# valette/FROG

Measured on AMD Instinct MI355X. Metric: registration iterations/sec (linear+deformable), higher is better.
Workload: dtype f32

## Files before the change

frog_amd/csrc/device/ctx.h:

```cpp
#pragma once

#include <hip/hip_runtime.h>

#include <cstdint>
#include <cstdio>
#include <cstring>
#include <string>
#include <memory>
#include <vector>

#include "../../../include/frog_hip.h"
#include "dev_buf.h"
#include "switches.h"

namespace frog {

extern thread_local std::string g_last_error;

inline int fail(int code, const std::string &msg)
{
    g_last_error = msg;
    return code;
}

#define FROG_HIP_CHECK(expr)                                                            \
    do {                                                                                \
        hipError_t e_ = (expr);                                                         \
        if (e_ != hipSuccess)                                                           \
            return ::frog::fail(FROG_E_HIP, std::string(#expr) + ": " + hipGetErrorString(e_)); \
    } while (0)

constexpr int SC_ENERGY = 0, SC_COUNT = 1;
constexpr int SC_OVERSIZE = 2;
constexpr int SC_LIST_STALE = 3;
constexpr int N_SCALARS = 4;
constexpr int HS_BBOX = 4, HS_SEQ = 7, HS_DOUBLES = 8;
struct ScalarHandoff {
    enum How { NONE, BY_KERNEL, BY_COPY, BY_COPY_SYNC } how = NONE;
    double seq = 0.0;
};
struct StepScalars {
    double E, n_oversize;
};


constexpr int TILE_POINTS = 256;
constexpr int N_XCD = 8;
constexpr int MAX_SUBPASS = 8;
constexpr int MAX_GROUPS = N_XCD * MAX_SUBPASS;
constexpr int REC_CHUNK = 128;
__host__ __device__ inline size_t group_sum_index(uint32_t group, uint32_t point, uint32_t own_points)
// ... 137 lines not shown
    frog::DevBuf<double> img_energy;
    frog::DevBuf<unsigned int> energy_ticket;
    double *h_energy = nullptr;
    double *h_energy_dev = nullptr;
    uint64_t scalar_seq = 0;

    bool deformable = false;
    frog::GridGeom geom{};
    frog::DevBuf<float4> coeff;
    frog::DevBuf<float4> grad;
    frog::DevBuf<float4> gradf;
    frog::DevBuf<float4> grad_spare;
    frog::DevBuf<uint32_t> lat_mask;
    frog::DevBuf<uint32_t> lat_inactive;
    frog::DevBuf<float4> ucoeff, ugrad, ugrad_spare;
    void commit_proposal() { coeff.swap(grad); ucoeff.swap(ugrad); coeff_zero = false; }
    void speculate_commit()
    {
        spec_coeff_zero = coeff_zero;
        coeff.swap(grad); grad.swap(grad_spare);
        ucoeff.swap(ugrad); ugrad.swap(ugrad_spare);
        coeff_zero = false;
    }
    void rollback_speculation()
    {
        grad.swap(grad_spare); coeff.swap(grad);
        ugrad.swap(ugrad_spare); ucoeff.swap(ugrad);
        coeff_zero = spec_coeff_zero;
    }
    frog::DevBuf<double> gridsum;
    frog::DevBuf<uint32_t> perm;
    frog::DevBuf<uint32_t> key_ptr;
    frog::DevBuf<uint32_t> key_cursor;
    frog::DevBuf<uint32_t> key_counts, brick_ptr_scratch, scan_sums;
    frog::DevBuf<unsigned char> scatter_blocks;
    frog::DevBuf<unsigned char> scatter_blocks_tmp;
    frog::DevBuf<uint32_t> len_hist;
    uint32_t n_scatter_blocks = 0;
    frog::DevBuf<float> bounds_scratch;
    frog::DevBuf<unsigned int> stray;
    uint32_t stray_parity = 0;
    bool centered_in_a = false;
    frog::DevBuf<long long> img_counts;
// ... 1 lines not shown
    std::vector<frog::GridRecord> grids;
    uint32_t n_hard = 0;
    float hard_weight2 = 0;
    frog::DevBuf<uint32_t> hl_point, hl_ptr, hl_partner;
    frog::DevBuf<double> hl_partial;
    frog::DevBuf<uint32_t> perm_tmp;
    frog::DevBuf<uint32_t> perm_key;
    frog::DevBuf<float4> scatter_stage;
    frog::DevBuf<uint32_t> brick_slot_ptr;
    frog::DevBuf<float4> extract_tmp;
    frog::DevBuf<uint32_t> subset_idx;
    frog::DevBuf<float> subset_out;
    std::vector<float4> h_res_sums, h_res_pos;
    bool res_valid = false;
    bool xyz2_fresh = false;
    float pending_alpha = 0;
    int phase = 0;

    bool ref_order = false;
    double create_s[3] = { 0, 0, 0 };
    int create_selections = 0;
    bool created = false;
    int lattice_reallocs = 0;
    bool two_collectives = false;
    bool finish_deformable = false;
    bool speculated = false;
    bool spec_coeff_zero = false;
    frog::ScalarHandoff pending;
    frog::DevBuf<uint32_t> ref_own;
    frog::DevBuf<float> ref_w, ref_d;
// ... 72 lines not shown
```

frog_amd/csrc/device/frog_hip.hip:

```cpp

#include "ctx.h"
#include <hip/hip_ext.h>
#include "prep.h"
#include "k_links.hip.h"
#include "k_stats.hip.h"
#include "k_grid.hip.h"
#include "k_comm.hip.h"
#include "k_cull.hip.h"
#include "k_ransac.hip.h"
#include "k_reforder.hip.h"
#include "k_refchain.hip.h"
#include "similarity.h"

#include <atomic>
#include <chrono>
#include <cmath>
#include <cstdlib>
#include <random>
#include <limits>
#include <new>

namespace frog {
thread_local std::string g_last_error;
constexpr int BOUNDS_BLOCKS = 256;
// ... 308 lines not shown
        ctx->pos_b_stale = false;
    }
    return FROG_OK;
}

static int post_step_scalars(frog_ctx *ctx, ScalarHandoff::How how, ScalarHandoff &h)
{
    h.how = how == ScalarHandoff::BY_KERNEL && !ctx->h_energy_dev ? ScalarHandoff::BY_COPY : how;
    h.seq = h.how == ScalarHandoff::BY_KERNEL ? (double)(++ctx->scalar_seq) : 0.0;
    if (h.how == ScalarHandoff::BY_KERNEL) return FROG_OK;
    FROG_HIP_CHECK(hipMemcpyAsync(ctx->h_energy, ctx->energy.p, N_SCALARS * sizeof(double), hipMemcpyDeviceToHost, ctx->stream));
    if (h.how == ScalarHandoff::BY_COPY) FROG_HIP_CHECK(hipEventRecord(ctx->energy_copied, ctx->stream));
    return FROG_OK;
}

static int await_step_scalars(frog_ctx *ctx, ScalarHandoff &h, StepScalars &out)
{
    const ScalarHandoff posted = h;
    h = ScalarHandoff{};
    volatile double *hs = ctx->h_energy;
    if (posted.how == ScalarHandoff::BY_KERNEL) {
        const auto t0 = std::chrono::steady_clock::now();
        unsigned spins = 0;
        while (hs[HS_SEQ] != posted.seq) {
            __builtin_ia32_pause();
            if ((++spins & 0xFFFFu) == 0u && std::chrono::steady_clock::now() - t0 > std::chrono::seconds(20)) {
                FROG_HIP_CHECK(hipStreamSynchronize(ctx->stream));
                if (hs[HS_SEQ] != posted.seq) return fail(FROG_E_HIP, "the step's scalars never arrived");
            }
        }
        std::atomic_thread_fence(std::memory_order_acquire);
    } else if (posted.how == ScalarHandoff::BY_COPY) FROG_HIP_CHECK(hipEventSynchronize(ctx->energy_copied));
    else FROG_HIP_CHECK(hipStreamSynchronize(ctx->stream));
    if (ctx->h_energy[SC_LIST_STALE] > 0) ctx->cull_need_build = true;
    out.E = std::sqrt(ctx->h_energy[SC_ENERGY] / ctx->h_energy[SC_COUNT]);
    out.n_oversize = ctx->h_energy[SC_OVERSIZE];
    return FROG_OK;
}

static bool step_rejected(const frog_ctx *ctx, double n_oversize) { return ctx->opt.guarantee_diffeomorphism && n_oversize > 0; }

static void record_displacement(frog_ctx *ctx, const P3 *out, bool measured, uint32_t n_blocks)
{
    if (measured) ctx->disp_n = ctx->disp_own_n = n_blocks;
    ctx->disp_others = false;
    ctx->disp_current = measured && out == ctx->pos2.p;
// ... 574 lines not shown
        for (uint32_t i = 0; i < c->n_owned(); i++) std::memcpy(&st[(size_t)i * MT_WORDS], x, sizeof x);
        CREATE_CHECK(c->mt_state.upload(st, s));
    }
    return FROG_OK;
}

static int create_solver_buffers(frog_ctx *c, const CreateClock &clock)
{
    hipStream_t s = c->stream;
    std::vector<double> hm((size_t)c->nI * 16, 0.0);
    for (uint32_t i = 0; i < c->nI; i++) for (int k = 0; k < 4; k++) hm[(size_t)i * 16 + 5 * k] = 1.0;
    CREATE_CHECK(c->mat.upload(hm, s));
    CREATE_CHECK(c->energy.alloc(4));
    CREATE_CHECK(c->energy_blocks.alloc(2 * ENERGY_BLOCKS));
    CREATE_CHECK(c->img_energy.alloc(2 * (size_t)std::max(1u, c->n_owned())));
    CREATE_CHECK(c->energy_ticket.alloc(2));
    CREATE_CHECK(hipMemsetAsync(c->energy_ticket.p, 0, 2 * sizeof(unsigned int), s));
    CREATE_CHECK(hipMemsetAsync(c->energy.p, 0, c->energy.bytes(), s));
    CREATE_CHECK(c->stray.alloc(3));
    CREATE_CHECK(hipMemsetAsync(c->stray.p, 0, 3 * sizeof(unsigned int), s));
    CREATE_CHECK(c->bounds_scratch.alloc((size_t)BOUNDS_BLOCKS * 6 + 6));
    em_derive_kernel<<<div_up(c->nI, 256), 256, 0, s>>>(c->em.p, c->emd.p, c->emf.p, c->nI, c->fast_theta());
    CREATE_CHECK(hipGetLastError());
    resolve_modes(c);
    CREATE_CHECK(c->cut_now.alloc(c->nI));
    CREATE_CHECK(c->lin_listed.alloc(1));
    CREATE_CHECK(hipMemsetAsync(c->lin_listed.p, 0, sizeof(unsigned long long), s));
    if (c->cull_enabled && (c->opt.inlier_threshold >= 1e-3f || c->cull_linear) && c->n_tiles > 0) {
        if (int rc_ = cull_allocate(c)) return rc_;
    }
    stats_publish_kernel<<<dim3(div_up(c->nI, 64), 2), 64, 0, s>>>(c->em.p, c->emd.p, c->emf.p, c->nI, c->opt.inlier_threshold, c->fast_theta(), c->cut_now.p, 1);
    CREATE_CHECK(hipGetLastError());
// ... 69 lines not shown
            (void)hipGetLastError();
        }
        if (c->retired_arena.alloc(arena) != hipSuccess) (void)hipGetLastError();
        c->retired_used = 0;
    }
    clock.lap("+ lattices allocated");
}

static void resolve_kernels(frog_ctx *c, const CreateClock &clock)
{
    const void *kernels[] = {
        (const void *)sweep_kernel<SWEEP_DEFORMABLE, true, false, false, false>, (const void *)sweep_kernel<SWEEP_DEFORMABLE, true, false, true, false>,
        (const void *)sweep_kernel<SWEEP_DEFORMABLE, true, false, false, true>, (const void *)sweep_kernel<SWEEP_COUNT, true, false, false, false>,
        (const void *)scatter_kernel, (const void *)lattice_step_kernel<true>, (const void *)lattice_step_kernel<false>,
        (const void *)transform_bspline_tile_kernel<float>, (const void *)transform_bspline_kernel<float>, (const void *)transform_bspline_kernel<float, 2>, (const void *)transform_zero_lattice_kernel,
        (const void *)cp_center_kernel, (const void *)bounds_kernel, (const void *)bounds_final_kernel, (const void *)zero_buffers_kernel,
        (const void *)brick_count_kernel, (const void *)brick_place_kernel, (const void *)cell_order_kernel, (const void *)brick_chunks_kernel,
        (const void *)scan_block_sums_kernel, (const void *)scan_of_sums_kernel, (const void *)scan_apply_kernel,
        (const void *)block_fill_kernel, (const void *)block_len_base_kernel, (const void *)block_sort_kernel,
        (const void *)cull_list_cutoff_kernel, (const void *)cull_allow_kernel, (const void *)cull_validate_kernel, (const void *)cull_disp_kernel,
        (const void *)count_reduce_kernel, (const void *)combine_groups_kernel, (const void *)energy_reduce_kernel,
        (const void *)lattice_step_kernel<true, LS_CPB_SMALL>, (const void *)lattice_step_kernel<false, LS_CPB_SMALL>,
        (const void *)stats_publish_kernel, (const void *)cull_allow_validate_kernel, (const void *)cull_count_kernel,
        (const void *)sweep_kernel<SWEEP_LINEAR, true, false, true, false>, (const void *)sweep_kernel<SWEEP_LINEAR, true, false, false, false>,
    };
    for (const void *k : kernels) { hipFuncAttributes fa; (void)hipFuncGetAttributes(&fa, k); }
    (void)hipGetLastError();
    scratch_warm_kernel<<<1, 64, 0, c->stream>>>(c->stray.p, 0);
    (void)hipGetLastError();
    (void)hipStreamSynchronize(c->stream);
    clock.lap("+ kernels resolved, stream idle");
// ... 153 lines not shown
            const float a = (float)((double)(1 - cpos) * lo + (double)cpos * hi);
            anchors[3 * (size_t)i + j] = a;
            if (i < nI - ctx->nf) average[j] += a / (float)(nI - ctx->nf);
        }
    std::vector<double> hm((size_t)nI * 16, 0.0);
    for (uint32_t i = 0; i < nI; i++) {
        for (int k = 0; k < 4; k++) hm[(size_t)i * 16 + 5 * k] = 1.0;
        for (int j = 0; j < 3; j++) hm[(size_t)i * 16 + 4 * j + 3] = (double)(average[j] - anchors[3 * (size_t)i + j]);
    }
    FROG_HIP_CHECK(hipMemcpyAsync(ctx->mat.p, hm.data(), hm.size() * sizeof(double), hipMemcpyHostToDevice, ctx->stream));
    FROG_HIP_CHECK(hipStreamSynchronize(ctx->stream));
    { const int rc = join_setup(ctx); if (rc) return rc; }
    ctx->deformable = false;
    ctx->phase = 0;
    ctx->xyz2_fresh = false; ctx->res_valid = false;
    ctx->disp_current = false; ctx->disp_spec = false; ctx->disp_others = false;
    ctx->cull_need_build = true; ctx->cull_check_due = true;
    stats_publish_kernel<<<dim3(div_up(ctx->nI, 64), 2), 64, 0, ctx->stream>>>(ctx->em.p, ctx->emd.p, ctx->emf.p, ctx->nI, ctx->opt.inlier_threshold, ctx->fast_theta(), ctx->cut_now.p, 1);
    FROG_HIP_CHECK(hipGetLastError());
    return FROG_OK;
}

static int launch_transform(frog_ctx *ctx, P3 *out, int apply, bool after_step = false, double scalar_seq = 0.0, double *trailer = nullptr)
{
    double *host_scalars = scalar_seq != 0.0 ? ctx->h_energy_dev : nullptr;
    const uint32_t n = ctx->own_pt_end - ctx->own_pt_begin;
    if (!n) return FROG_OK;
    Span span(ctx, FROG_K_TRANSFORM);
    if (!ctx->deformable) {
        const bool with_disp = cull_active_linear(ctx) && ctx->cull_lin_builds > 0 && !ctx->cull_need_build && ctx->pos2_snap.p;
        transform_linear_kernel<<<div_up(n, 256), 256, 0, ctx->stream>>>(ctx->pos.p, out, ctx->mat.p,
                                                                        ctx->own_pt_begin, ctx->own_pt_end, apply,
                                                                        with_disp ? ctx->pos2_snap.p : nullptr, ctx->disp_part.p,
                                                                        ctx->disp_allow.p, ctx->cull_state.p, ctx->energy.p,
                                                                        host_scalars, scalar_seq, trailer);
        trailer = nullptr;
        record_displacement(ctx, out, with_disp, div_up(n, 256));
    } else if (ctx->coeff_zero && !after_step) {
        record_displacement(ctx, out, false, 0);
        transform_zero_lattice_kernel<<<div_up(n, 256), 256, 0, ctx->stream>>>(ctx->pos.p, out, ctx->own_pt_begin, ctx->own_pt_end, apply);
    } else if (ctx->ref_order) {
        { const int rc = join_setup(ctx); if (rc) return rc; }
        record_displacement(ctx, out, false, 0);
        ref_transform_bspline_kernel<<<div_up(n, 256), 256, 0, ctx->stream>>>(ctx->pos.p, out, ctx->coeff.p, ctx->own_pt_begin, ctx->own_pt_end,
                                                                             ctx->ib, to_dev(ctx->geom), apply, after_step ? ctx->grad.p : nullptr,
                                                                             ctx->energy.p, ctx->opt.guarantee_diffeomorphism, host_scalars, scalar_seq);
    } else {
        { const int rc = join_setup_positions(ctx); if (rc) return rc; }
        const bool with_disp = cull_active(ctx) && ctx->cull_builds > 0 && !ctx->cull_need_build;
        const bool tiled = ctx->n_scatter_blocks > 0 && ctx->geom.brick == 4 && !ctx->sw.k11_pointwise
                           && (n >= 1000000u || ctx->sw.k11_tiled);
        if (tiled) {
            const GeomDev gd = to_dev(ctx->geom);
            const size_t lds = (size_t)K11_TILE_ENTRIES * sizeof(float4);
            auto kernel = ctx->sw.k11_f64 ? transform_bspline_tile_kernel<double> : transform_bspline_tile_kernel<float>;
// ... 13 lines not shown
            const bool pt_xcd = ctx->sw.k11_point_by_xcd >= 0 ? ctx->sw.k11_point_by_xcd != 0 : nb >= 8192u;
            kernel<<<pt_xcd ? ((nb + 7u) & ~7u) : nb, 256, 0, ctx->stream>>>(ctx->pos.p, ctx->pos_b.p, out, ctx->coeff.p,
                                                                             ctx->perm.p, n, ctx->ib, to_dev(ctx->geom), apply,
                                                                             with_disp ? ctx->pos2_snap.p : nullptr, ctx->disp_part.p,
                                                                             after_step ? ctx->grad.p : nullptr, ctx->energy.p,
                                                                             ctx->opt.guarantee_diffeomorphism,
                                                                             ctx->disp_allow.p, ctx->cull_state.p, host_scalars, scalar_seq, trailer,
                                                                             pt_xcd ? nb : 0u);
            record_displacement(ctx, out, with_disp, nb);
        }
        trailer = nullptr;
    }
    if (trailer) slab_trailer_kernel<<<1, 1, 0, ctx->stream>>>(ctx->energy.p, trailer);
    FROG_HIP_CHECK(hipGetLastError());
    if (apply) { ctx->pos_b_stale = true; ctx->rc_valid = false; }
    return FROG_OK;
}

int frog_transform_points_local(frog_ctx *ctx, int apply)
{
    CTX_GUARD(ctx);
    const uint32_t n = ctx->own_pt_end - ctx->own_pt_begin;
    if (!n) return FROG_OK;
    if (ctx->xyz2_fresh && !apply) {
        ctx->xyz2_fresh = false; ctx->res_valid = false;
        ctx->disp_current = ctx->disp_spec;
        if (ctx->n_owned() == ctx->nI && !ctx->xyz2_exported && ctx->pos2_spec.n == ctx->pos2.n) {
            std::swap(ctx->pos2.p, ctx->pos2_spec.p);
            std::swap(ctx->pos2.cap, ctx->pos2_spec.cap);
            return FROG_OK;
        }
        FROG_HIP_CHECK(hipMemcpyAsync(ctx->pos2.p + ctx->own_pt_begin, ctx->pos2_spec.p + ctx->own_pt_begin,
                                      (size_t)n * sizeof(P3), hipMemcpyDeviceToDevice, ctx->stream));
        return FROG_OK;
    }
    ctx->xyz2_fresh = false; ctx->res_valid = false;
    return launch_transform(ctx, ctx->pos2.p, apply);
}

int frog_transform_points(frog_ctx *ctx, int apply) { return frog_transform_points_local(ctx, apply); }

int frog_update_stats_local(frog_ctx *ctx)
{
    CTX_GUARD(ctx);
    const uint32_t nO = ctx->n_owned();
    const uint32_t cap = (uint32_t)ctx->sample_cap;
    hipStream_t s = ctx->stream;
    const int cur = (int)(ctx->sel_consumed % (uint64_t)ctx->sel_ring);
    FROG_HIP_CHECK(hipStreamWaitEvent(s, ctx->sel_done[cur], 0));
    {
        Span span(ctx, FROG_K_STATS);
// ... 27 lines not shown
    if (!ctx->deformable) ctx->cull_need_build = true;
    ctx->cull_check_due = true;
    FROG_HIP_CHECK(hipGetLastError());
    return FROG_OK;
}

int frog_update_stats(frog_ctx *ctx)
{
    if (ctx && !ctx->whole_group())
        return fail(FROG_E_STATE, "context owns a sub-range of images: use frog_update_stats_local + all-reduce + frog_stats_publish");
    int rc = frog_update_stats_local(ctx);
    if (rc) return rc;
    if (ctx->helper) {
        frog_ctx *h = ctx->helper;
        const size_t n = ctx->own_pt_end - ctx->own_pt_begin;
        FROG_HIP_CHECK(hipMemcpyAsync(h->pos2.p + ctx->own_pt_begin, ctx->pos2.p + ctx->own_pt_begin, n * sizeof(P3),
                                      hipMemcpyDeviceToDevice, ctx->stream));
        rc = frog_update_stats_local(h);
        if (rc) return rc;
        FROG_HIP_CHECK(hipMemcpyAsync(ctx->em.p, h->em.p, (size_t)ctx->nf * sizeof(float4), hipMemcpyDeviceToDevice, ctx->stream));
    }
    return frog_stats_publish(ctx);
}

int frog_ransac(frog_ctx *ctx, const frog_model *m, uint32_t image, const frog_ransac_options *o, int64_t *n_inliers)
{
    CTX_GUARD(ctx);
    if (!m || !o) return fail(FROG_E_INVALID, "null argument");
    if (image < ctx->ib || image >= ctx->ie) return fail(FROG_E_INVALID, "image not owned by this context");
    if (m->n_images != ctx->nI || m->point_offset[ctx->nI] != ctx->P) return fail(FROG_E_INVALID, "model does not match the context");
// ... 79 lines not shown
        const float *in = m->xyz + 3 * ((size_t)pb + pt);
        const float t[3] = { (float)(best[0] * in[0] + best[1] * in[1] + best[2] * in[2] + best[3]),
                             (float)(best[4] * in[0] + best[5] * in[1] + best[6] * in[2] + best[7]),
                             (float)(best[8] * in[0] + best[9] * in[1] + best[10] * in[2] + best[11]) };
        for (uint64_t l = m->row_ptr[pb + pt]; l < m->row_ptr[pb + pt + 1]; l++) {
            const float *pB = &xyz2[3 * ((size_t)m->point_offset[m->link_image[l]] + m->link_point[l])];
            const float dx = t[0] - pB[0], dy = t[1] - pB[1], dz = t[2] - pB[2];
            if (dx * dx + dy * dy + dz * dz < maxDistance2) { srcs.push_back(in); tgts.push_back(pB); }
        }
    }
    double fit[16];
    if (!frog::similarity_fit(srcs.size(), [&](size_t i, double a[3], double b[3]) {
            for (int k = 0; k < 3; k++) { a[k] = srcs[i][k]; b[k] = tgts[i][k]; }
        }, fit))
        std::memcpy(fit, best, sizeof fit);
    FROG_HIP_CHECK(hipMemcpyAsync(ctx->mat.p + (size_t)image * 16, fit, sizeof fit, hipMemcpyHostToDevice, s));
    FROG_HIP_CHECK(hipStreamSynchronize(s));
    if (n_inliers) *n_inliers = maxNumberOfInliers;
    return FROG_OK;
}

int frog_linear_step_local(frog_ctx *ctx)
{
    CTX_GUARD(ctx);
    if (ctx->deformable) return fail(FROG_E_STATE, "linear step after deformable set-up");
    if (ctx->ref_order) { ctx->xyz2_fresh = false; return ref_linear_step(ctx); }
    hipStream_t s = ctx->stream;
    bool culled = cull_active_linear(ctx);
    ctx->build_in_sweep = false;
    if (culled) {
        Span span(ctx, FROG_K_CULL);
        const int rc = cull_prepare(ctx);
        if (rc) return rc;
        culled = cull_active_linear(ctx);
    }
    {
        Span span(ctx, ctx->build_in_sweep ? FROG_K_SWEEP_LINEAR_BUILD : FROG_K_SWEEP_LINEAR, ctx->n_sub == 1);
        for (uint32_t sub = 0; sub < ctx->n_sub; sub++)
            launch_sweep<SWEEP_LINEAR>(ctx, sub, s, span.attached ? span.a : nullptr, span.attached ? span.b : nullptr, culled,
                                       ctx->build_in_sweep);
// ... 21 lines not shown

int frog_linear_step(frog_ctx *ctx, double *E)
{
    int rc = frog_linear_step_local(ctx);
    if (rc) return rc;
    const uint32_t n = ctx->own_pt_end - ctx->own_pt_begin;
    if (!(ctx->whole_group() && ctx->h_energy_dev && n && !ctx->helper))
        return frog_energy_read(ctx, E, nullptr);
    if (ctx->pos2_spec.n != ctx->P) FROG_HIP_CHECK(ctx->pos2_spec.alloc(ctx->P));
    ScalarHandoff h; StepScalars sc;
    rc = post_step_scalars(ctx, ScalarHandoff::BY_KERNEL, h);
    if (rc) return rc;
    rc = launch_transform(ctx, ctx->pos2_spec.p, 0, false, h.seq);
    if (rc) return rc;
    ctx->xyz2_fresh = true;
    rc = await_step_scalars(ctx, h, sc);
    if (rc) return rc;
    if (E) *E = sc.E;
    return FROG_OK;
}

int frog_bounds_local(frog_ctx *ctx, double mins[3], double maxs[3])
{
    CTX_GUARD(ctx);
    hipStream_t s = ctx->stream;
    bounds_kernel<<<BOUNDS_BLOCKS, 256, 0, s>>>(ctx->pos.p, ctx->own_pt_begin, ctx->own_pt_end, ctx->bounds_scratch.p);
    bounds_final_kernel<<<1, 256, 0, s>>>(ctx->bounds_scratch.p, BOUNDS_BLOCKS, ctx->bounds_scratch.p + (size_t)BOUNDS_BLOCKS * 6);
    FROG_HIP_CHECK(hipGetLastError());
    float *h = reinterpret_cast<float *>(ctx->h_energy + HS_BBOX);
    FROG_HIP_CHECK(hipMemcpyAsync(h, ctx->bounds_scratch.p + (size_t)BOUNDS_BLOCKS * 6, 6 * sizeof(float), hipMemcpyDeviceToHost, s));
    FROG_HIP_CHECK(hipStreamSynchronize(s));
    for (int k = 0; k < 3; k++) { mins[k] = (double)h[k]; maxs[k] = (double)h[3 + k]; }
    return FROG_OK;
}


static int make_geometry(const frog_ctx *ctx, int level, const double mins[3], const double maxs[3], GridGeom &g, frog_grid_info &info)
{
    const double size = (double)ctx->opt.initial_grid_size / std::pow(2, level);
    const float sc = 1 + 2 * ctx->opt.bounding_box_margin;
// ... 109 lines not shown
            FROG_HIP_CHECK(gr.kept_mask->alloc_async(std::max<size_t>(1, mask_words), ctx->stream));
            FROG_HIP_CHECK(gr.kept_u->alloc_async(std::max<size_t>(1, G), ctx->stream));
        }
        FROG_HIP_CHECK(hipMemcpyAsync(gr.kept_mask->p, ctx->lat_mask.p, mask_words * sizeof(uint32_t), hipMemcpyDeviceToDevice, ctx->stream));
        FROG_HIP_CHECK(hipMemcpyAsync(gr.kept_u->p, ctx->ucoeff.p, G * sizeof(float4), hipMemcpyDeviceToDevice, ctx->stream));
    }
    gr.retired = true;
    return FROG_OK;
}

int frog_deformable_setup_bounds(frog_ctx *ctx, int level, const double mins[3], const double maxs[3], frog_grid_info *out)
{
    CTX_GUARD(ctx);
    if (level < 0 || level > 30) return fail(FROG_E_INVALID, "bad level");
    ctx->xyz2_fresh = false; ctx->res_valid = false; ctx->rc_valid = false;
    const auto t_setup = std::chrono::steady_clock::now();
    auto setup_lap = [&](const char *what) {
        if (ctx->sw.setup_trace) std::fprintf(stderr, "[setup level %d] %-28s %9.3f ms\n", level, what, std::chrono::duration<double, std::milli>(std::chrono::steady_clock::now() - t_setup).count());
    };
    int rc = join_setup(ctx);
    if (rc) return rc;
    setup_lap("joined the last set-up");
    rc = retire_current_grid(ctx);
    if (rc) return rc;
    setup_lap("+ finished lattice retired");

    GridGeom g{};
    frog_grid_info info{};
    rc = make_geometry(ctx, level, mins, maxs, g, info);
    if (rc) return rc;
// ... 252 lines not shown

int frog_deformable_phase_c(frog_ctx *ctx, double *E)
{
    CTX_GUARD(ctx);
    if (ctx->phase != 2) return fail(FROG_E_STATE, "phase_c without phase_b");
    ScalarHandoff h; StepScalars sc;
    int rc = post_step_scalars(ctx, ctx->own_pt_end > ctx->own_pt_begin ? ScalarHandoff::BY_KERNEL : ScalarHandoff::BY_COPY, h);
    if (rc) return rc;
    rc = launch_transform(ctx, ctx->pos2_spec.p, 0, true, h.seq);
    if (rc) return rc;
    ctx->xyz2_fresh = true;
    rc = await_step_scalars(ctx, h, sc);
    if (rc) return rc;
    const bool rejected = step_rejected(ctx, sc.n_oversize);
    if (!rejected) ctx->commit_proposal();
    ctx->phase = 0;
    if (E) *E = rejected ? -1.0 : sc.E;
    return FROG_OK;
}

int frog_deformable_step(frog_ctx *ctx, float alpha, double *E)
{
    if (ctx && !ctx->whole_group())
        return fail(FROG_E_STATE, "context owns a sub-range of images: use the phase_a/b/c entry points");
    int rc = frog_deformable_phase_a(ctx, alpha);
    if (rc) return rc;
    rc = frog_deformable_phase_b(ctx);
    if (rc) return rc;
    return frog_deformable_phase_c(ctx, E);
}
// ... 29 lines not shown
    CTX_GUARD(ctx);
    int rc = FROG_OK;
    if (xyz) rc = download_points(ctx, ctx->pos.p, xyz);
    if (!rc && xyz2) rc = download_points(ctx, ctx->pos2.p, xyz2);
    return rc;
}

int frog_set_points2(frog_ctx *ctx, const float *xyz2)
{
    CTX_GUARD(ctx);
    if (!xyz2) return fail(FROG_E_INVALID, "null input");
    std::vector<P3> h(ctx->P);
    for (size_t p = 0; p < ctx->P; p++)
        h[ctx->h_new_of_old[p]] = P3{ xyz2[3 * p], xyz2[3 * p + 1], xyz2[3 * p + 2] };
    ctx->xyz2_fresh = false; ctx->res_valid = false; ctx->disp_current = false;
    FROG_HIP_CHECK(hipMemcpyAsync(ctx->pos2.p, h.data(), h.size() * sizeof(P3), hipMemcpyHostToDevice, ctx->stream));
    FROG_HIP_CHECK(hipStreamSynchronize(ctx->stream));
    return FROG_OK;
}

__global__ void gather_points_kernel(const P3 *pos2, const uint32_t *idx, uint32_t n, float *out)
{
    const uint32_t i = blockIdx.x * blockDim.x + threadIdx.x;
    if (i >= n) return;
    const P3 p = pos2[idx[i]];
    out[3 * i] = p.x; out[3 * i + 1] = p.y; out[3 * i + 2] = p.z;
}

int frog_get_points2_subset(frog_ctx *ctx, const uint64_t *points, size_t n, float *xyz2)
{
// ... 508 lines not shown
    const bool carried = sum_mask && ctx->h_energy_dev;
    if (sum_mask) {
        a.sum_mask = sum_mask; a.energy = ctx->energy.p;
        if (carried) {
            const int rc = post_step_scalars(ctx, ScalarHandoff::BY_KERNEL, ctx->pending);
            if (rc) return rc;
            a.host_scalars = ctx->h_energy_dev; a.seq = ctx->pending.seq;
        }
        ctx->finish_deformable = ctx->phase == 2;
    }
    const dim3 grid((unsigned)std::min<uint64_t>(std::max<uint64_t>(div_up(longest, 256), 1), 1024), world);
    if (own_rows_too) { ctx->disp_current = ctx->disp_spec; ctx->disp_spec = false; }
    const bool list = ctx->deformable ? (cull_active(ctx) && ctx->cull_builds > 0) : (cull_active_linear(ctx) && ctx->cull_lin_builds > 0);
    const bool measure = ctx->disp_current && list && !ctx->cull_need_build && ctx->pos2_snap.p && ctx->disp_part.p
                         && (size_t)ctx->disp_own_n + (size_t)grid.x * grid.y <= ctx->disp_part.n;
    unpack_slab_kernel<<<grid, 256, 0, ctx->stream>>>(reinterpret_cast<const P3 *>(slab), ctx->pos2.p, a,
                                                      measure ? ctx->pos2_snap.p : nullptr, measure ? ctx->disp_part.p + ctx->disp_own_n : nullptr);
    FROG_HIP_CHECK(hipGetLastError());
    record_displacement_others(ctx, measure, grid.x * grid.y);
    if (sum_mask && !carried) return post_step_scalars(ctx, ScalarHandoff::BY_COPY, ctx->pending);
    return FROG_OK;
}

int frog_comm_unpack_slab(frog_ctx *ctx, const void *slab, uint64_t slot_rows, uint32_t world_size, const uint64_t *row_begin, uint32_t self)
{
    return unpack_slab(ctx, slab, slot_rows, world_size, row_begin, self, 0, false);
}

int frog_comm_mode(frog_ctx *ctx, int two_collectives)
{
// ... 68 lines not shown
    } else {
        if (ctx->phase != 2) return fail(FROG_E_STATE, "frog_step_finish: no deformable step pending");
        if (!rejected) ctx->commit_proposal();
        ctx->phase = 0;
    }
    if (E) *E = rejected ? -1.0 : sc.E;
    return FROG_OK;
}

int frog_comm_buffer(frog_ctx *ctx, int which, void **ptr, size_t *bytes, size_t *row_begin, size_t *row_end)
{
    CTX_GUARD(ctx);
    size_t b = 0, rb = 0, re = 0;
    void *p = nullptr;
    switch (which) {
    case FROG_BUF_XYZ2: ctx->xyz2_exported = true; ctx->disp_current = false; p = ctx->pos2.p; b = ctx->pos2.bytes(); rb = ctx->own_pt_begin; re = ctx->own_pt_end; break;
    case FROG_BUF_EM: p = ctx->em.p; b = ctx->em.bytes(); rb = ctx->ib; re = ctx->ie; break;
    case FROG_BUF_ENERGY: p = ctx->energy.p; b = ctx->energy.bytes(); rb = 0; re = 4; break;
    case FROG_BUF_GRIDSUM:
        if (!ctx->deformable) return fail(FROG_E_STATE, "no lattice");
        p = ctx->gridsum.p; re = 3 * (size_t)ctx->geom.n_cp + (ctx->two_collectives ? 4 : 0); b = re * sizeof(double); rb = 0; break;
    default: return fail(FROG_E_INVALID, "unknown buffer");
    }
    if (ptr) *ptr = p;
    if (bytes) *bytes = b;
    if (row_begin) *row_begin = rb;
    if (row_end) *row_end = re;
    return FROG_OK;
}

}
// ... 1 lines not shown
```

frog_amd/csrc/device/k_grid.hip.h:

```cpp
#pragma once

#include "ctx.h"

namespace frog {

struct GeomDev {
    int dims[3];
    int n_cp;
    double origin[3];
    double spacing[3];
    double inv_spacing[3];
    int brick;
    int nbricks[3];
    int n_bricks;
    int lat_sh;
    uint32_t lat_mask;
    size_t lat_blk, lat_img;
    uint32_t mask_words;
};

__device__ __forceinline__ bool lat_active(const uint32_t *mask, const GeomDev &g, uint32_t img, uint32_t node)
{
    return (mask[(size_t)img * g.mask_words + (node >> 5)] >> (node & 31u)) & 1u;
}
// ... 305 lines not shown
    float mn[3] = { 3.402823466e38f, 3.402823466e38f, 3.402823466e38f };
    float mx[3] = { -3.402823466e38f, -3.402823466e38f, -3.402823466e38f };
    for (int b = threadIdx.x; b < n_blocks; b += 256)
        for (int k = 0; k < 3; k++) { mn[k] = fminf(mn[k], block_minmax[b * 6 + k]); mx[k] = fmaxf(mx[k], block_minmax[b * 6 + 3 + k]); }
    for (int k = 0; k < 3; k++) { sh[k][threadIdx.x] = mn[k]; sh[3 + k][threadIdx.x] = mx[k]; }
    __syncthreads();
    for (int h = 128; h > 0; h >>= 1) {
        if ((int)threadIdx.x < h)
            for (int k = 0; k < 3; k++) {
                sh[k][threadIdx.x] = fminf(sh[k][threadIdx.x], sh[k][threadIdx.x + h]);
                sh[3 + k][threadIdx.x] = fmaxf(sh[3 + k][threadIdx.x], sh[3 + k][threadIdx.x + h]);
            }
        __syncthreads();
    }
    if (threadIdx.x < 6) out6[threadIdx.x] = sh[threadIdx.x][0];
}

__device__ __forceinline__ void scatter_cell(const float in[3], const GeomDev &g, int ic[3], float frac[3])
{
    #pragma unroll
    for (int k = 0; k < 3; k++) {
        const float coord = (float)(((double)in[k] - g.origin[k]) / g.spacing[k]);
        const int c = (int)floorf(coord);
        ic[k] = c;
        frac[k] = coord - (float)c;
    }
}

constexpr int BRICK_BLOCK_POINTS = 1024;
constexpr int BRICK_LDS_KEYS = 8192;
// ... 1066 lines not shown
```

frog_amd/csrc/device/switches.h:

```cpp
#pragma once

#include <algorithm>
#include <cstdint>
#include <cstdio>
#include <cstdlib>

namespace frog {

struct Switches {
    bool wide_records = false;
    int subpasses = 1;
    int tile_slices = 0;
    int fused = -1;
    bool scalars_copy = false;
    bool cull = true;
    bool cull_linear = true;
    float cull_scale = 2.0f, cull_pad = 25.0f;
    float cull_lin_scale = 1.25f, cull_lin_pad = 10.0f;
    bool cull_build_pass = false;
    bool weight_exact = false;
    bool weight_general = false;
    int reference_order = -1;
    bool ref_literal = false;
    uint32_t rc_grid_x = 1u << 22;
    bool ref_trace = false;
    bool k11_f64 = false;
    bool k11_pointwise = false, k11_tiled = false;
    int k11_by_xcd = -1;
    int k11_point_by_xcd = -1;
    int brick = 0;
    int lattice_blocked = -1, lattice_sparse = -1;
    bool energy_pass = false;
    bool timing = false;
    bool setup_trace = false;
};

inline Switches read_switches(int max_subpasses)
{
    Switches sw;
    auto on = [](const char *e, bool unset) { return e ? atoi(e) != 0 : unset; };
    auto tri = [](const char *e) { return e ? (atoi(e) != 0 ? 1 : 0) : -1; };
    auto skin = [](const char *e, float &scale, float &pad) {
        float a = 0, b = 0;
        if (e && sscanf(e, "%f,%f", &a, &b) == 2 && a >= 1.0f && b >= 0.0f) { scale = a; pad = b; }
    };
    const char *e;
    e = getenv("FROG_WIDE_RECORDS"); sw.wide_records = e && e[0] == '1';
// ... 9 lines not shown
    sw.weight_exact = on(getenv("FROG_WEIGHT_EXACT"), false);
    sw.weight_general = on(getenv("FROG_WEIGHT_GENERAL"), false);
    sw.reference_order = tri(getenv("FROG_REFERENCE_ORDER"));
    sw.ref_literal = getenv("FROG_REF_LITERAL") != nullptr;
    if ((e = getenv("FROG_RC_GRID_X"))) sw.rc_grid_x = (uint32_t)std::max(1, atoi(e));
    sw.ref_trace = getenv("FROG_REF_TRACE") != nullptr;
    sw.k11_f64 = on(getenv("FROG_K11_F64"), false);
    sw.k11_pointwise = getenv("FROG_K11_POINTWISE") != nullptr;
    sw.k11_tiled = getenv("FROG_K11_TILED") != nullptr;
    if ((e = getenv("FROG_K11_BY_XCD"))) sw.k11_by_xcd = atoi(e);
    if ((e = getenv("FROG_K11_POINT_BY_XCD"))) sw.k11_point_by_xcd = atoi(e);
    if ((e = getenv("FROG_BRICK"))) { const int b = atoi(e); if (b == 4 || b == 8) sw.brick = b; }
    sw.lattice_blocked = tri(getenv("FROG_LATTICE_BLOCKED"));
    sw.lattice_sparse = tri(getenv("FROG_LATTICE_SPARSE"));
    sw.energy_pass = getenv("FROG_ENERGY_PASS") != nullptr;
    sw.timing = getenv("FROG_TIMING") != nullptr;
    sw.setup_trace = getenv("FROG_SETUP_TRACE") != nullptr;
    return sw;
}

}
```

Measured before the change: 2503.

## Rebase positions by copying standing pos2 and publish bounds from the same kernel

Adds state flags that record when pos2 already holds the transformed positions for the current transform. When an apply-transform is requested in that state, a single rebase kernel copies pos2 into pos and computes the bounding box in the same pass, instead of re-running the transform. The bounding box is written to pinned host memory so the later bounds query only waits on a sequence number and skips its own two kernels. It also skips the zero-lattice transform when pos2 already equals pos. The cost is a lot of invalidation bookkeeping across many entry points, and any missed case would leave stale positions.

```diff
diff --git a/frog_amd/csrc/device/ctx.h b/frog_amd/csrc/device/ctx.h
--- a/frog_amd/csrc/device/ctx.h
+++ b/frog_amd/csrc/device/ctx.h
@@ -34,7 +34,7 @@
 constexpr int SC_OVERSIZE = 2;
 constexpr int SC_LIST_STALE = 3;
 constexpr int N_SCALARS = 4;
-constexpr int HS_BBOX = 4, HS_SEQ = 7, HS_DOUBLES = 8;
+constexpr int HS_BBOX = 4, HS_SEQ = 7, HS_REBASE_BBOX = 8, HS_REBASE_SEQ = 11, HS_DOUBLES = 12;
 struct ScalarHandoff {
     enum How { NONE, BY_KERNEL, BY_COPY, BY_COPY_SYNC } how = NONE;
     double seq = 0.0;
@@ -202,19 +202,21 @@
     frog::DevBuf<uint32_t> lat_mask;
     frog::DevBuf<uint32_t> lat_inactive;
     frog::DevBuf<float4> ucoeff, ugrad, ugrad_spare;
-    void commit_proposal() { coeff.swap(grad); ucoeff.swap(ugrad); coeff_zero = false; }
+    void commit_proposal() { coeff.swap(grad); ucoeff.swap(ugrad); coeff_zero = false; transform_changed(); }
     void speculate_commit()
     {
         spec_coeff_zero = coeff_zero;
         coeff.swap(grad); grad.swap(grad_spare);
         ucoeff.swap(ugrad); ugrad.swap(ugrad_spare);
         coeff_zero = false;
+        transform_changed();
     }
     void rollback_speculation()
     {
         grad.swap(grad_spare); coeff.swap(grad);
         ugrad.swap(ugrad_spare); ucoeff.swap(ugrad);
         coeff_zero = spec_coeff_zero;
+        transform_changed();
     }
     frog::DevBuf<double> gridsum;
     frog::DevBuf<uint32_t> perm;
@@ -246,6 +248,11 @@
     std::vector<float4> h_res_sums, h_res_pos;
     bool res_valid = false;
     bool xyz2_fresh = false;
+    bool pos2_standing = false, spec_standing = false, pos2_is_pos = false, rebase_bounds_current = false;
+    uint64_t rebase_seq = 0;
+    void transform_changed() { pos2_standing = false; spec_standing = false; }
+    void pos2_changed() { pos2_standing = false; pos2_is_pos = false; }
+    void pos_changed() { pos2_standing = false; spec_standing = false; pos2_is_pos = false; rebase_bounds_current = false; }
     float pending_alpha = 0;
     int phase = 0;
 
diff --git a/frog_amd/csrc/device/frog_hip.hip b/frog_amd/csrc/device/frog_hip.hip
--- a/frog_amd/csrc/device/frog_hip.hip
+++ b/frog_amd/csrc/device/frog_hip.hip
@@ -346,22 +346,29 @@
     return FROG_OK;
 }
 
+static int await_pinned_seq(frog_ctx *ctx, int hs_slot, double seq, const char *what)
+{
+    volatile double *hs = ctx->h_energy;
+    const auto t0 = std::chrono::steady_clock::now();
+    unsigned spins = 0;
+    while (hs[hs_slot] != seq) {
+        __builtin_ia32_pause();
+        if ((++spins & 0xFFFFu) == 0u && std::chrono::steady_clock::now() - t0 > std::chrono::seconds(20)) {
+            FROG_HIP_CHECK(hipStreamSynchronize(ctx->stream));
+            if (hs[hs_slot] != seq) return fail(FROG_E_HIP, what);
+        }
+    }
+    std::atomic_thread_fence(std::memory_order_acquire);
+    return FROG_OK;
+}
+
 static int await_step_scalars(frog_ctx *ctx, ScalarHandoff &h, StepScalars &out)
 {
     const ScalarHandoff posted = h;
     h = ScalarHandoff{};
-    volatile double *hs = ctx->h_energy;
     if (posted.how == ScalarHandoff::BY_KERNEL) {
-        const auto t0 = std::chrono::steady_clock::now();
-        unsigned spins = 0;
-        while (hs[HS_SEQ] != posted.seq) {
-            __builtin_ia32_pause();
-            if ((++spins & 0xFFFFu) == 0u && std::chrono::steady_clock::now() - t0 > std::chrono::seconds(20)) {
-                FROG_HIP_CHECK(hipStreamSynchronize(ctx->stream));
-                if (hs[HS_SEQ] != posted.seq) return fail(FROG_E_HIP, "the step's scalars never arrived");
-            }
-        }
-        std::atomic_thread_fence(std::memory_order_acquire);
+        const int rc = await_pinned_seq(ctx, HS_SEQ, posted.seq, "the step's scalars never arrived");
+        if (rc) return rc;
     } else if (posted.how == ScalarHandoff::BY_COPY) FROG_HIP_CHECK(hipEventSynchronize(ctx->energy_copied));
     else FROG_HIP_CHECK(hipStreamSynchronize(ctx->stream));
     if (ctx->h_energy[SC_LIST_STALE] > 0) ctx->cull_need_build = true;
@@ -966,8 +973,8 @@
     CREATE_CHECK(c->energy.alloc(4));
     CREATE_CHECK(c->energy_blocks.alloc(2 * ENERGY_BLOCKS));
     CREATE_CHECK(c->img_energy.alloc(2 * (size_t)std::max(1u, c->n_owned())));
-    CREATE_CHECK(c->energy_ticket.alloc(2));
-    CREATE_CHECK(hipMemsetAsync(c->energy_ticket.p, 0, 2 * sizeof(unsigned int), s));
+    CREATE_CHECK(c->energy_ticket.alloc(3));
+    CREATE_CHECK(hipMemsetAsync(c->energy_ticket.p, 0, 3 * sizeof(unsigned int), s));
     CREATE_CHECK(hipMemsetAsync(c->energy.p, 0, c->energy.bytes(), s));
     CREATE_CHECK(c->stray.alloc(3));
     CREATE_CHECK(hipMemsetAsync(c->stray.p, 0, 3 * sizeof(unsigned int), s));
@@ -1067,7 +1074,7 @@
         (const void *)sweep_kernel<SWEEP_DEFORMABLE, true, false, false, true>, (const void *)sweep_kernel<SWEEP_COUNT, true, false, false, false>,
         (const void *)scatter_kernel, (const void *)lattice_step_kernel<true>, (const void *)lattice_step_kernel<false>,
         (const void *)transform_bspline_tile_kernel<float>, (const void *)transform_bspline_kernel<float>, (const void *)transform_bspline_kernel<float, 2>, (const void *)transform_zero_lattice_kernel,
-        (const void *)cp_center_kernel, (const void *)bounds_kernel, (const void *)bounds_final_kernel, (const void *)zero_buffers_kernel,
+        (const void *)cp_center_kernel, (const void *)bounds_kernel, (const void *)bounds_final_kernel, (const void *)rebase_kernel, (const void *)zero_buffers_kernel,
         (const void *)brick_count_kernel, (const void *)brick_place_kernel, (const void *)cell_order_kernel, (const void *)brick_chunks_kernel,
         (const void *)scan_block_sums_kernel, (const void *)scan_of_sums_kernel, (const void *)scan_apply_kernel,
         (const void *)block_fill_kernel, (const void *)block_len_base_kernel, (const void *)block_sort_kernel,
@@ -1251,6 +1258,7 @@
     ctx->deformable = false;
     ctx->phase = 0;
     ctx->xyz2_fresh = false; ctx->res_valid = false;
+    ctx->transform_changed();
     ctx->disp_current = false; ctx->disp_spec = false; ctx->disp_others = false;
     ctx->cull_need_build = true; ctx->cull_check_due = true;
     stats_publish_kernel<<<dim3(div_up(ctx->nI, 64), 2), 64, 0, ctx->stream>>>(ctx->em.p, ctx->emd.p, ctx->emf.p, ctx->nI, ctx->opt.inlier_threshold, ctx->fast_theta(), ctx->cut_now.p, 1);
@@ -1264,6 +1272,7 @@
     const uint32_t n = ctx->own_pt_end - ctx->own_pt_begin;
     if (!n) return FROG_OK;
     Span span(ctx, FROG_K_TRANSFORM);
+    bool wrote_out = true;
     if (!ctx->deformable) {
         const bool with_disp = cull_active_linear(ctx) && ctx->cull_lin_builds > 0 && !ctx->cull_need_build && ctx->pos2_snap.p;
         transform_linear_kernel<<<div_up(n, 256), 256, 0, ctx->stream>>>(ctx->pos.p, out, ctx->mat.p,
@@ -1275,7 +1284,8 @@
         record_displacement(ctx, out, with_disp, div_up(n, 256));
     } else if (ctx->coeff_zero && !after_step) {
         record_displacement(ctx, out, false, 0);
-        transform_zero_lattice_kernel<<<div_up(n, 256), 256, 0, ctx->stream>>>(ctx->pos.p, out, ctx->own_pt_begin, ctx->own_pt_end, apply);
+        if (out == ctx->pos2.p && ctx->pos2_is_pos) wrote_out = false;
+        else transform_zero_lattice_kernel<<<div_up(n, 256), 256, 0, ctx->stream>>>(ctx->pos.p, out, ctx->own_pt_begin, ctx->own_pt_end, apply);
     } else if (ctx->ref_order) {
         { const int rc = join_setup(ctx); if (rc) return rc; }
         record_displacement(ctx, out, false, 0);
@@ -1319,6 +1329,29 @@
     if (trailer) slab_trailer_kernel<<<1, 1, 0, ctx->stream>>>(ctx->energy.p, trailer);
     FROG_HIP_CHECK(hipGetLastError());
     if (apply) { ctx->pos_b_stale = true; ctx->rc_valid = false; }
+    if (apply && wrote_out) ctx->pos_changed();
+    else if (out == ctx->pos2.p && wrote_out) ctx->pos2_changed();
+    ctx->pos2_standing = out == ctx->pos2.p && !apply && !after_step && !ctx->ref_order;
+    if (out != ctx->pos2.p) ctx->spec_standing = false;
+    return FROG_OK;
+}
+
+static bool rebase_by_copy(const frog_ctx *ctx)
+{
+    return ctx->pos2_standing && !ctx->sw.boundary_legacy && ctx->whole_group() && !ctx->ref_order && !ctx->xyz2_exported;
+}
+static int launch_rebase(frog_ctx *ctx)
+{
+    Span span(ctx, FROG_K_TRANSFORM);
+    float *host6 = ctx->h_energy_dev ? reinterpret_cast<float *>(ctx->h_energy_dev + HS_REBASE_BBOX) : nullptr;
+    const double seq = (double)(++ctx->rebase_seq);
+    rebase_kernel<<<BOUNDS_BLOCKS, 256, 0, ctx->stream>>>(ctx->pos.p, ctx->pos2.p, ctx->own_pt_begin, ctx->own_pt_end, ctx->bounds_scratch.p,
+                                                          ctx->energy_ticket.p + 2, host6, host6 ? ctx->h_energy_dev + HS_REBASE_SEQ : nullptr, seq);
+    FROG_HIP_CHECK(hipGetLastError());
+    ctx->pos_b_stale = true; ctx->rc_valid = false;
+    ctx->pos_changed();
+    ctx->pos2_is_pos = ctx->deformable && !ctx->sw.k11_f64;
+    ctx->rebase_bounds_current = host6 != nullptr;
     return FROG_OK;
 }
 
@@ -1330,6 +1363,8 @@
     if (ctx->xyz2_fresh && !apply) {
         ctx->xyz2_fresh = false; ctx->res_valid = false;
         ctx->disp_current = ctx->disp_spec;
+        ctx->pos2_changed();
+        ctx->pos2_standing = ctx->spec_standing;
         if (ctx->n_owned() == ctx->nI && !ctx->xyz2_exported && ctx->pos2_spec.n == ctx->pos2.n) {
             std::swap(ctx->pos2.p, ctx->pos2_spec.p);
             std::swap(ctx->pos2.cap, ctx->pos2_spec.cap);
@@ -1340,6 +1375,7 @@
         return FROG_OK;
     }
     ctx->xyz2_fresh = false; ctx->res_valid = false;
+    if (apply && rebase_by_copy(ctx)) return launch_rebase(ctx);
     return launch_transform(ctx, ctx->pos2.p, apply);
 }
 
@@ -1397,6 +1433,7 @@
     if (ctx->helper) {
         frog_ctx *h = ctx->helper;
         const size_t n = ctx->own_pt_end - ctx->own_pt_begin;
+        h->pos2_changed();
         FROG_HIP_CHECK(hipMemcpyAsync(h->pos2.p + ctx->own_pt_begin, ctx->pos2.p + ctx->own_pt_begin, n * sizeof(P3),
                                       hipMemcpyDeviceToDevice, ctx->stream));
         rc = frog_update_stats_local(h);
@@ -1506,6 +1543,7 @@
             for (int k = 0; k < 3; k++) { a[k] = srcs[i][k]; b[k] = tgts[i][k]; }
         }, fit))
         std::memcpy(fit, best, sizeof fit);
+    ctx->transform_changed();
     FROG_HIP_CHECK(hipMemcpyAsync(ctx->mat.p + (size_t)image * 16, fit, sizeof fit, hipMemcpyHostToDevice, s));
     FROG_HIP_CHECK(hipStreamSynchronize(s));
     if (n_inliers) *n_inliers = maxNumberOfInliers;
@@ -1516,6 +1554,7 @@
 {
     CTX_GUARD(ctx);
     if (ctx->deformable) return fail(FROG_E_STATE, "linear step after deformable set-up");
+    ctx->transform_changed();
     if (ctx->ref_order) { ctx->xyz2_fresh = false; return ref_linear_step(ctx); }
     hipStream_t s = ctx->stream;
     bool culled = cull_active_linear(ctx);
@@ -1567,6 +1606,7 @@
     rc = launch_transform(ctx, ctx->pos2_spec.p, 0, false, h.seq);
     if (rc) return rc;
     ctx->xyz2_fresh = true;
+    ctx->spec_standing = !ctx->ref_order;
     rc = await_step_scalars(ctx, h, sc);
     if (rc) return rc;
     if (E) *E = sc.E;
@@ -1577,6 +1617,13 @@
 {
     CTX_GUARD(ctx);
     hipStream_t s = ctx->stream;
+    if (ctx->rebase_bounds_current && !ctx->sw.boundary_legacy) {
+        const int rc = await_pinned_seq(ctx, HS_REBASE_SEQ, (double)ctx->rebase_seq, "the re-base's bounding box never arrived");
+        if (rc) return rc;
+        const float *hb = reinterpret_cast<const float *>(ctx->h_energy + HS_REBASE_BBOX);
+        for (int k = 0; k < 3; k++) { mins[k] = (double)hb[k]; maxs[k] = (double)hb[3 + k]; }
+        return FROG_OK;
+    }
     bounds_kernel<<<BOUNDS_BLOCKS, 256, 0, s>>>(ctx->pos.p, ctx->own_pt_begin, ctx->own_pt_end, ctx->bounds_scratch.p);
     bounds_final_kernel<<<1, 256, 0, s>>>(ctx->bounds_scratch.p, BOUNDS_BLOCKS, ctx->bounds_scratch.p + (size_t)BOUNDS_BLOCKS * 6);
     FROG_HIP_CHECK(hipGetLastError());
@@ -1716,6 +1763,7 @@
     CTX_GUARD(ctx);
     if (level < 0 || level > 30) return fail(FROG_E_INVALID, "bad level");
     ctx->xyz2_fresh = false; ctx->res_valid = false; ctx->rc_valid = false;
+    ctx->transform_changed();
     const auto t_setup = std::chrono::steady_clock::now();
     auto setup_lap = [&](const char *what) {
         if (ctx->sw.setup_trace) std::fprintf(stderr, "[setup level %d] %-28s %9.3f ms\n", level, what, std::chrono::duration<double, std::milli>(std::chrono::steady_clock::now() - t_setup).count());
@@ -1998,6 +2046,7 @@
     if (rc) return rc;
     const bool rejected = step_rejected(ctx, sc.n_oversize);
     if (!rejected) ctx->commit_proposal();
+    ctx->spec_standing = !ctx->ref_order && ctx->own_pt_end > ctx->own_pt_begin;
     ctx->phase = 0;
     if (E) *E = rejected ? -1.0 : sc.E;
     return FROG_OK;
@@ -2057,6 +2106,7 @@
     for (size_t p = 0; p < ctx->P; p++)
         h[ctx->h_new_of_old[p]] = P3{ xyz2[3 * p], xyz2[3 * p + 1], xyz2[3 * p + 2] };
     ctx->xyz2_fresh = false; ctx->res_valid = false; ctx->disp_current = false;
+    ctx->pos2_changed();
     FROG_HIP_CHECK(hipMemcpyAsync(ctx->pos2.p, h.data(), h.size() * sizeof(P3), hipMemcpyHostToDevice, ctx->stream));
     FROG_HIP_CHECK(hipStreamSynchronize(ctx->stream));
     return FROG_OK;
@@ -2595,6 +2645,7 @@
     const bool list = ctx->deformable ? (cull_active(ctx) && ctx->cull_builds > 0) : (cull_active_linear(ctx) && ctx->cull_lin_builds > 0);
     const bool measure = ctx->disp_current && list && !ctx->cull_need_build && ctx->pos2_snap.p && ctx->disp_part.p
                          && (size_t)ctx->disp_own_n + (size_t)grid.x * grid.y <= ctx->disp_part.n;
+    ctx->pos2_changed();
     unpack_slab_kernel<<<grid, 256, 0, ctx->stream>>>(reinterpret_cast<const P3 *>(slab), ctx->pos2.p, a,
                                                       measure ? ctx->pos2_snap.p : nullptr, measure ? ctx->disp_part.p + ctx->disp_own_n : nullptr);
     FROG_HIP_CHECK(hipGetLastError());
@@ -2693,7 +2744,7 @@
     size_t b = 0, rb = 0, re = 0;
     void *p = nullptr;
     switch (which) {
-    case FROG_BUF_XYZ2: ctx->xyz2_exported = true; ctx->disp_current = false; p = ctx->pos2.p; b = ctx->pos2.bytes(); rb = ctx->own_pt_begin; re = ctx->own_pt_end; break;
+    case FROG_BUF_XYZ2: ctx->xyz2_exported = true; ctx->disp_current = false; ctx->pos2_changed(); p = ctx->pos2.p; b = ctx->pos2.bytes(); rb = ctx->own_pt_begin; re = ctx->own_pt_end; break;
     case FROG_BUF_EM: p = ctx->em.p; b = ctx->em.bytes(); rb = ctx->ib; re = ctx->ie; break;
     case FROG_BUF_ENERGY: p = ctx->energy.p; b = ctx->energy.bytes(); rb = 0; re = 4; break;
     case FROG_BUF_GRIDSUM:
diff --git a/frog_amd/csrc/device/k_grid.hip.h b/frog_amd/csrc/device/k_grid.hip.h
--- a/frog_amd/csrc/device/k_grid.hip.h
+++ b/frog_amd/csrc/device/k_grid.hip.h
@@ -343,6 +343,80 @@
         __syncthreads();
     }
     if (threadIdx.x < 6) out6[threadIdx.x] = sh[threadIdx.x][0];
+}
+
+__global__ __launch_bounds__(256) void rebase_kernel(float4 *pos, const P3 *pos2, uint32_t pt_begin, uint32_t pt_end,
+                                                     float *block_minmax , unsigned int *ticket,
+                                                     float *host6, double *host_seq, double seq)
+{
+    __shared__ float sh[6][256];
+    __shared__ int last_s;
+    float mn[3] = { 3.402823466e38f, 3.402823466e38f, 3.402823466e38f };
+    float mx[3] = { -3.402823466e38f, -3.402823466e38f, -3.402823466e38f };
+    constexpr int AHEAD = 8;
+    const uint64_t stride = (uint64_t)gridDim.x * blockDim.x;
+    uint64_t p = (uint64_t)pt_begin + blockIdx.x * blockDim.x + threadIdx.x;
+    for (; p + (AHEAD - 1) * stride < pt_end; p += AHEAD * stride) {
+        P3 v[AHEAD];
+        #pragma unroll
+        for (int u = 0; u < AHEAD; u++) v[u] = pos2[p + u * stride];
+        #pragma unroll
+        for (int u = 0; u < AHEAD; u++) {
+            *reinterpret_cast<P3 *>(&pos[p + u * stride]) = v[u];
+            mn[0] = fminf(mn[0], v[u].x); mn[1] = fminf(mn[1], v[u].y); mn[2] = fminf(mn[2], v[u].z);
+            mx[0] = fmaxf(mx[0], v[u].x); mx[1] = fmaxf(mx[1], v[u].y); mx[2] = fmaxf(mx[2], v[u].z);
+        }
+    }
+    for (; p < pt_end; p += stride) {
+        const P3 v = pos2[p];
+        *reinterpret_cast<P3 *>(&pos[p]) = v;
+        mn[0] = fminf(mn[0], v.x); mn[1] = fminf(mn[1], v.y); mn[2] = fminf(mn[2], v.z);
+        mx[0] = fmaxf(mx[0], v.x); mx[1] = fmaxf(mx[1], v.y); mx[2] = fmaxf(mx[2], v.z);
+    }
+    for (int k = 0; k < 3; k++) { sh[k][threadIdx.x] = mn[k]; sh[3 + k][threadIdx.x] = mx[k]; }
+    __syncthreads();
+    for (int h = 128; h > 0; h >>= 1) {
+        if ((int)threadIdx.x < h)
+            for (int k = 0; k < 3; k++) {
+                sh[k][threadIdx.x] = fminf(sh[k][threadIdx.x], sh[k][threadIdx.x + h]);
+                sh[3 + k][threadIdx.x] = fmaxf(sh[3 + k][threadIdx.x], sh[3 + k][threadIdx.x + h]);
+            }
+        __syncthreads();
+    }
+    if (threadIdx.x == 0) {
+        for (int k = 0; k < 6; k++) __hip_atomic_store(&block_minmax[blockIdx.x * 6 + k], sh[k][0], __ATOMIC_RELAXED, __HIP_MEMORY_SCOPE_AGENT);
+        __threadfence();
+        last_s = atomicAdd(ticket, 1u) == gridDim.x - 1u;
+    }
+    __syncthreads();
+    if (!last_s) return;
+    __threadfence();
+    for (int k = 0; k < 3; k++) { mn[k] = 3.402823466e38f; mx[k] = -3.402823466e38f; }
+    for (int b = threadIdx.x; b < (int)gridDim.x; b += 256)
+        for (int k = 0; k < 3; k++) {
+            mn[k] = fminf(mn[k], __hip_atomic_load(&block_minmax[b * 6 + k], __ATOMIC_RELAXED, __HIP_MEMORY_SCOPE_AGENT));
+            mx[k] = fmaxf(mx[k], __hip_atomic_load(&block_minmax[b * 6 + 3 + k], __ATOMIC_RELAXED, __HIP_MEMORY_SCOPE_AGENT));
+        }
+    for (int k = 0; k < 3; k++) { sh[k][threadIdx.x] = mn[k]; sh[3 + k][threadIdx.x] = mx[k]; }
+    __syncthreads();
+    for (int h = 128; h > 0; h >>= 1) {
+        if ((int)threadIdx.x < h)
+            for (int k = 0; k < 3; k++) {
+                sh[k][threadIdx.x] = fminf(sh[k][threadIdx.x], sh[k][threadIdx.x + h]);
+                sh[3 + k][threadIdx.x] = fmaxf(sh[3 + k][threadIdx.x], sh[3 + k][threadIdx.x + h]);
+            }
+        __syncthreads();
+    }
+    if (threadIdx.x == 0) {
+        float *out6 = block_minmax + (size_t)gridDim.x * 6;
+        for (int k = 0; k < 6; k++) out6[k] = sh[k][0];
+        *ticket = 0u;
+        if (host6) {
+            for (int k = 0; k < 6; k++) __hip_atomic_store(&host6[k], sh[k][0], __ATOMIC_RELAXED, __HIP_MEMORY_SCOPE_SYSTEM);
+            __threadfence_system();
+            __hip_atomic_store(host_seq, seq, __ATOMIC_RELEASE, __HIP_MEMORY_SCOPE_SYSTEM);
+        }
+    }
 }
 
 __device__ __forceinline__ void scatter_cell(const float in[3], const GeomDev &g, int ic[3], float frac[3])
diff --git a/frog_amd/csrc/device/switches.h b/frog_amd/csrc/device/switches.h
--- a/frog_amd/csrc/device/switches.h
+++ b/frog_amd/csrc/device/switches.h
@@ -31,6 +31,7 @@
     int brick = 0;
     int lattice_blocked = -1, lattice_sparse = -1;
     bool energy_pass = false;
+    bool boundary_legacy = false;
     bool timing = false;
     bool setup_trace = false;
 };
@@ -70,6 +71,7 @@
     sw.lattice_blocked = tri(getenv("FROG_LATTICE_BLOCKED"));
     sw.lattice_sparse = tri(getenv("FROG_LATTICE_SPARSE"));
     sw.energy_pass = getenv("FROG_ENERGY_PASS") != nullptr;
+    sw.boundary_legacy = on(getenv("FROG_BOUNDARY_LEGACY"), false);
     sw.timing = getenv("FROG_TIMING") != nullptr;
     sw.setup_trace = getenv("FROG_SETUP_TRACE") != nullptr;
     return sw;
```

New measurement: 2504 (median of 4 runs). About the same (+0.0%).
